# OCR-D/ocrd_keraslm

Hardware: AMD Instinct MI355X
Metric: chars/sec training (stacked-LSTM forward+backward+Adam) (higher is better)
Workload: dtype bf16; 1 GPU; cfg2: depth=2 width=512 length=256 V=256 1 context, stateful training, 3072 streams/GPU, synthetic 10M-char corpus (SURVEY.md 8d); streams_per_gpu=3072, global_batch=3072, seq_len=256, parallelism=dp1

## Files before the change

include/keraslm_hip.h:

```cpp
#ifndef KERASLM_HIP_H
#define KERASLM_HIP_H

#include <stddef.h>
#include <stdint.h>

#ifdef __cplusplus
extern "C" {
#endif

#define KL_ABI_VERSION 1

enum {
  KL_OK = 0,
  KL_ERR_SHAPE = 1,
  KL_ERR_LAUNCH = 2,
  KL_ERR_STATE = 3,
  KL_ERR_WORKSPACE = 4,
  KL_ERR_ARG = 5
};

#define KL_PREC_BF16 1
#define KL_PREC_SPLIT 3

typedef struct kl_config {
// ... 44 lines not shown
int kl_step_batch(kl_handle* h, int n, const int32_t* idx, const int32_t* ctx, float* pool, const int32_t* slot_in,
                  const int32_t* slot_out, float* probs, void* ws, size_t ws_bytes, void* stream);

void* kl_host_alloc(size_t bytes);
void kl_host_free(void* p);
size_t kl_step_host_workspace_bytes(const kl_handle* h, int n);
int kl_step_batch_host(kl_handle* h, int n, const int32_t* idx, const int32_t* ctx, const int32_t* slot_in,
                       const int32_t* slot_out, const int32_t* target, float* pool, int head_k, float* probs_host,
                       float* heads_host, uint32_t* done_host, uint32_t ticket, void* ws, size_t ws_bytes, void* stream);
int kl_step_wait(const uint32_t* done_host, uint32_t ticket, double timeout_s);

int kl_state_dist2(const kl_handle* h, int n, const float* pool, const int32_t* a, const int32_t* b, int k,
                   float* out, void* stream);

int kl_trace_enable(kl_handle* h, int on);
int kl_trace_read(kl_handle* h, int kind, int* n_launches, float* total_ms, int* persistent,
                  double* flops_per_launch);
const char* kl_trace_kernel_name(kl_handle* h, int kind);

int kl_test_gemm_tn(const uint16_t* A, const uint16_t* B, void* C, const float* bias, int M, int N, int K, long lda,
                    long ldb, long ldc, int out_mode, int splits, void* stream);
int kl_test_gemm_an(const uint16_t* A_km, const uint16_t* B, float* C, int M, int N, int K, long lda_km, long ldb,
                    long ldc, int c_transposed, int b_km, void* stream);
int kl_test_thin_gemm(const float* A, long lda, const uint16_t* WT_hi, const uint16_t* WT_lo, long ldw, int M, int N,
                      int K, float* C, long ldc, int split, void* stream);

#ifdef __cplusplus
}
#endif
#endif
```

ocrd_keraslm_amd/csrc/api.hip:

```cpp
#include <hip/hip_runtime.h>
#include <stdio.h>
#include <stdlib.h>
#include <string.h>
#include <time.h>

#include <functional>
#include <utility>

#include <vector>

#include "kl_common.h"
#include "kl_kernels.h"

namespace {

inline size_t align_up(size_t x, size_t a) { return (x + a - 1) / a * a; }
inline int round_up_i(int x, int a) { return (x + a - 1) / a * a; }

struct Carver {
  unsigned char* base;
  size_t off = 0;
  explicit Carver(void* b) : base(reinterpret_cast<unsigned char*>(b)) {}
  template <typename T>
  T* take(size_t count) {
// ... 1205 lines not shown
    } else if (dz_km) {
      KL_TRY(kl_launch_gemm_an(w.dZ[l], (const bf16_t*)w.H[l], grads + h->off_U[l], 4 * W, W, BT, 4 * W, W, 4 * W, 1, s, 1));
    } else if (w.ht_ready) {
      KL_TRY(kl_launch_gemm_tn(w.HTf[l], w.dZT, grads + h->off_U[l], nullptr, W, 4 * W, BT, ldtf, BTp, 4 * W, 2, ksplit, 1.f, s));
    } else {
      KL_TRY(kl_launch_transpose_bf16((const bf16_t*)w.H[l], W, w.HT, BTp, BT, W, s));
      KL_TRY(kl_launch_gemm_tn(w.HT, w.dZT, grads + h->off_U[l], nullptr, W, 4 * W, BTp, BTp, BTp, 4 * W, 2, ksplit, 1.f, s));
    }
    if (!db_done) KL_TRY(kl_launch_colsum_bf16(w.dZ[l], 4 * W, BT, 4 * W, grads + h->off_b[l], s));
    if (l > 0) {
      const bool masked_in = masks != nullptr && (l - 1) > 0;
      const bf16_t* X = masked_in ? w.Hd[l - 1] : (const bf16_t*)w.H[l - 1] + BW;
      if (pair_uk) {
      } else if (dz_km) {
        KL_TRY(kl_launch_gemm_an(w.dZ[l], X, grads + h->off_K[l], 4 * W, W, BT, 4 * W, W, 4 * W, 1, s, 1));
      } else if (w.ht_ready) {
        const bf16_t* XT = masked_in ? w.HdT[l - 1] : w.HTf[l - 1] + B;
        KL_TRY(kl_launch_gemm_tn(XT, w.dZT, grads + h->off_K[l], nullptr, W, 4 * W, BT, masked_in ? (long)BT : ldtf, BTp, 4 * W, 2, ksplit, 1.f, s));
      } else {
        KL_TRY(kl_launch_transpose_bf16(X, W, w.HT, BTp, BT, W, s));
        KL_TRY(kl_launch_gemm_tn(w.HT, w.dZT, grads + h->off_K[l], nullptr, W, 4 * W, BTp, BTp, BTp, 4 * W, 2, ksplit, 1.f, s));
      }
    } else {
      if (kl_launch_onehot_dense(idx, B, T, Vp, 0, 1, w.OHT, BTp, s) == KL_ERR_SHAPE) {
        KL_TRY(kl_zero_async(w.OHT, (size_t)Vp * BTp * sizeof(bf16_t), s));
        KL_TRY(kl_launch_onehot_t(idx, B, T, V, 0, 1, w.OHT, BTp, s));
      }
      KL_TRY(kl_zero_async(w.dEKT, (size_t)4 * W * Vp * sizeof(float), s));
      bool pair_ctx = dz_km && h->fuse_wg && c.n_ctx >= 1 && (Vp % 128) == 0 &&
                      kl_gemm_an_applicable(4 * W, Vp + c.ctx_vocab, BT, 4 * W);
      if (pair_ctx) {
        if (kl_launch_onehot_dense(ctx, B, T, c.ctx_vocab, 0, c.n_ctx, w.OHC[0], BTp, s) == KL_ERR_SHAPE) {
          KL_TRY(kl_zero_async(w.OHC[0], (size_t)c.ctx_vocab * BTp * sizeof(bf16_t), s));
          KL_TRY(kl_launch_onehot_t(ctx, B, T, c.ctx_vocab, 0, c.n_ctx, w.OHC[0], BTp, s));
        }
        KL_TRY(kl_zero_async(w.dCtxKT[0], (size_t)4 * W * c.ctx_vocab * sizeof(float), s));
        const int pe = kl_launch_gemm_an2(w.dZ[l], w.OHT, w.dEKT, 4 * W, Vp, BT, 4 * W, BTp, Vp, 0,
                                          w.OHC[0], w.dCtxKT[0], c.ctx_vocab, BTp, c.ctx_vocab, 0, s, 0);
        if (pe == KL_ERR_SHAPE) pair_ctx = false;
        else KL_TRY(pe);
      }
      if (pair_ctx) {
      } else if (dz_km) KL_TRY(kl_launch_gemm_an(w.dZ[l], w.OHT, w.dEKT, 4 * W, Vp, BT, 4 * W, BTp, Vp, 0, s));
      else KL_TRY(kl_launch_gemm_tn(w.dZT, w.OHT, w.dEKT, nullptr, 4 * W, Vp, BTp, BTp, BTp, Vp, 2, ksplit, 1.f, s));
      KL_TRY(kl_launch_f32_to_bf16_t(w.dEKT, Vp, 4 * W, Vp, w.dEKT_bf, nullptr, Vp, 0, s));
      KL_TRY(kl_launch_f32_to_bf16_t(w.dEKT, Vp, 4 * W, Vp, w.dEK_bf, nullptr, 4 * W, 1, s));
      KL_TRY(kl_launch_gemm_tn(d.ET, w.dEKT_bf, grads + h->off_K[0], nullptr, W, 4 * W, Vp, Vp, Vp, 4 * W, 0, 1, 1.f, s));
      KL_TRY(kl_launch_gemm_tn(w.dEK_bf, d.Kn[0], grads + h->off_E, nullptr, V, W, 4 * W, 4 * W, 4 * W, W, 2, 1, 1.f, s));
      for (int n = 0; n < c.n_ctx; ++n) {
        if (!(pair_ctx && n == 0)) {
          if (kl_launch_onehot_dense(ctx, B, T, c.ctx_vocab, n, c.n_ctx, w.OHC[n], BTp, s) == KL_ERR_SHAPE) {
            KL_TRY(kl_zero_async(w.OHC[n], (size_t)c.ctx_vocab * BTp * sizeof(bf16_t), s));
            KL_TRY(kl_launch_onehot_t(ctx, B, T, c.ctx_vocab, n, c.n_ctx, w.OHC[n], BTp, s));
          }
          KL_TRY(kl_zero_async(w.dCtxKT[n], (size_t)4 * W * c.ctx_vocab * sizeof(float), s));
          if (dz_km) KL_TRY(kl_launch_gemm_an(w.dZ[l], w.OHC[n], w.dCtxKT[n], 4 * W, c.ctx_vocab, BT, 4 * W, BTp, c.ctx_vocab, 0, s));
          else KL_TRY(kl_launch_gemm_tn(w.dZT, w.OHC[n], w.dCtxKT[n], nullptr, 4 * W, c.ctx_vocab, BTp, BTp, BTp,
                                        c.ctx_vocab, 2, ksplit, 1.f, s));
        }
        const size_t krow = (size_t)(W + n * c.ctx_dim) * 4 * W;
        KL_TRY(kl_launch_ctx_grads(P + h->off_Ctx[n], P + h->off_K[0] + krow, 4 * W, c.ctx_vocab, c.ctx_dim,
                                   w.dCtxKT[n], c.ctx_vocab, 4 * W, grads + h->off_K[0] + krow, 4 * W,
                                   grads + h->off_Ctx[n], s));
      }
    }
      return 0;
// ... 538 lines not shown
  }
}

int kl_state_dist2(const kl_handle* h, int n, const float* pool, const int32_t* a, const int32_t* b, int k, float* out,
                   void* stream) {
  if (!h || !pool || !a || !b || !out || n < 1) return KL_ERR_ARG;
  if (k < 0 || k >= 2 * h->cfg.depth) return KL_ERR_ARG;
  const int W = h->cfg.width;
  hipLaunchKernelGGL(state_dist2_kernel, dim3((n + 3) / 4), dim3(256), 0, (hipStream_t)stream, pool,
                     (long)2 * h->cfg.depth * W, W, k, a, b, n, out);
  return hip_ok(hipGetLastError());
}

int kl_test_gemm_tn(const uint16_t* A, const uint16_t* B, void* C, const float* bias, int M, int N, int K, long lda,
                    long ldb, long ldc, int out_mode, int splits, void* stream) {
  return kl_launch_gemm_tn(A, B, C, bias, M, N, K, lda, ldb, ldc, out_mode, splits, 1.f, (hipStream_t)stream);
}

int kl_test_gemm_an(const uint16_t* A_km, const uint16_t* B, float* C, int M, int N, int K, long lda_km, long ldb,
                    long ldc, int c_transposed, int b_km, void* stream) {
  return kl_launch_gemm_an(A_km, B, C, M, N, K, lda_km, ldb, ldc, c_transposed, (hipStream_t)stream, b_km);
}

int kl_test_thin_gemm(const float* A, long lda, const uint16_t* WT_hi, const uint16_t* WT_lo, long ldw, int M, int N,
                      int K, float* C, long ldc, int split, void* stream) {
  KlOperand op;
  memset(&op, 0, sizeof(op));
  op.A = A; op.lda = lda; op.a_is_f32 = 1; op.WT_hi = WT_hi; op.WT_lo = WT_lo; op.ldw = ldw; op.K = K;
  return kl_launch_thin_gemm(&op, M, N, C, ldc, nullptr, split, (hipStream_t)stream);
}

}

extern "C" int kl_test_fwd_step(const uint16_t* A, long lda, const uint16_t* WT, long ldw, int K, int n_ops,
                                int n_rows, int W, int fused, int iters, float* c_out, uint16_t* h_out,
                                void* stream) {
  KlFwdStep st[4];
  if (fused < 1 || fused > 4 || n_ops < 1 || n_ops > 2) return KL_ERR_ARG;
  for (int f = 0; f < fused; ++f) {
    KlFwdStep& S = st[f];
    memset(&S, 0, sizeof(S));
    S.n_rows = n_rows; S.W = W; S.split = 1; S.n_ops = n_ops;
    for (int p = 0; p < n_ops; ++p) {
      KlOperand& o = S.op[p];
      o.A = A; o.lda = lda; o.WT_hi = WT + (size_t)(f * 2 + p) * (size_t)4 * W * ldw; o.ldw = ldw;
      o.K = K; o.a_is_f32 = 0;
// ... 143 lines not shown
```

ocrd_keraslm_amd/csrc/elementwise.hip:

```cpp
#include <string.h>

#include "kl_common.h"
#include "kl_kernels.h"

namespace {

struct CtxTabs { const float* t[8]; };

__global__ void embed_gather_kernel(const float* __restrict__ E, CtxTabs tabs, int n_ctx, int ctx_dim, int W,
                                    const int* __restrict__ idx, const int* __restrict__ ctx, int B, int T,
                                    bf16_t* __restrict__ X, long ldx, int Dp) {
  const int chunks = Dp >> 3;
  const long total = (long)B * T * chunks;
  for (long e = blockIdx.x * (long)blockDim.x + threadIdx.x; e < total; e += (long)gridDim.x * blockDim.x) {
    const int c = (int)(e % chunks);
    const long row = e / chunks;
    const int b = (int)(row % B), t = (int)(row / B);
    const int id = idx[(long)b * T + t];
    frag16 o;
#pragma unroll
    for (int j = 0; j < 8; ++j) {
      const int d = c * 8 + j;
      float v = 0.f;
      if (d < W) {
// ... 272 lines not shown
                                    bf16_t* __restrict__ out, long ld) {
  const long r0 = ((long)blockIdx.x * blockDim.x + threadIdx.x) * 8;
  if (r0 >= ld) return;
  const long total = (long)B * T;
  int id[8];
#pragma unroll
  for (int j = 0; j < 8; ++j) {
    const long r = r0 + j;
    id[j] = -1;
    if (r < total) {
      const int b = (int)(r % B), t = (int)(r / B);
      id[j] = ids[((long)b * T + t) * n_cols + col];
    }
  }
  const int v0 = blockIdx.y * 32;
  for (int v = v0; v < v0 + 32 && v < n_rows; ++v) {
    uint4 w;
    w.x = (id[0] == v ? 0x3F80u : 0u) | (id[1] == v ? 0x3F800000u : 0u);
    w.y = (id[2] == v ? 0x3F80u : 0u) | (id[3] == v ? 0x3F800000u : 0u);
    w.z = (id[4] == v ? 0x3F80u : 0u) | (id[5] == v ? 0x3F800000u : 0u);
    w.w = (id[6] == v ? 0x3F80u : 0u) | (id[7] == v ? 0x3F800000u : 0u);
    *reinterpret_cast<uint4*>(out + (long)v * ld + r0) = w;
  }
}

__global__ void reg_stats_kernel(const float* __restrict__ X, int R, int D, float* __restrict__ scratch) {
  extern __shared__ float sm[];
  float* col = sm;
  float* red = sm + D;
  const int tid = threadIdx.x, nt = blockDim.x;
  float* mean = scratch;
  float* s1 = scratch + D;
  float* s2 = scratch + 2 * D;
  float* nr = scratch + 3 * D;
  for (int d = tid; d < D; d += nt) col[d] = 0.f;
  __syncthreads();
  if (D <= nt) {
    const int ng = nt / D, g = tid / D, d = tid % D;
    if (g < ng) {
      float a = 0.f;
#pragma unroll 8
      for (int r = 1 + g; r < R; r += ng) a += X[(long)r * D + d];
      atomicAdd(&col[d], a);
    }
  } else {
    for (int d = tid; d < D; d += nt) {
// ... 204 lines not shown

int kl_launch_adam(float* p, const float* g, float* m, float* v, size_t n, float lr_t, float b1, float b2,
                   float eps, float clip, float grad_scale, hipStream_t stream) {
  hipLaunchKernelGGL(adam_kernel, dim3(grid_for((long)n, 256)), dim3(256), 0, stream, p, g, m, v, n, lr_t, b1, b2,
                     eps, clip, grad_scale);
  return ok();
}

int kl_launch_onehot_t(const int* ids, int B, int T, int n_classes, int col, int n_cols, bf16_t* out, long ld,
                       hipStream_t stream) {
  hipLaunchKernelGGL(onehot_t_kernel, dim3(grid_for((long)B * T, 256)), dim3(256), 0, stream, ids, B, T, n_classes,
                     col, n_cols, out, ld);
  return ok();
}

int kl_launch_onehot_dense(const int* ids, int B, int T, int n_rows, int col, int n_cols, bf16_t* out, long ld,
                           hipStream_t stream) {
  if ((ld & 7) || ((size_t)out & 15) || ld < (long)B * T) return KL_ERR_SHAPE;
  dim3 grid((unsigned)((ld / 8 + 255) / 256), (unsigned)((n_rows + 31) / 32));
  hipLaunchKernelGGL(onehot_dense_kernel, grid, dim3(256), 0, stream, ids, B, T, n_rows, col, n_cols, out, ld);
  return ok();
}

int kl_launch_regulariser_grads(const float* E, int V, int W, const float* const* ctx_tabs, int n_ctx, int ctx_vocab,
                                int ctx_dim, float* gE, float* const* gCtx, float* loss_acc, float* scratch,
                                hipStream_t stream) {
  const int nt = 1024;
  if (V >= 2) {
    const size_t lds = (size_t)(W + 2 * nt) * sizeof(float);
    if (lds > 64 * 1024) return KL_ERR_SHAPE;
    hipLaunchKernelGGL(reg_stats_kernel, dim3(1), dim3(nt), lds, stream, E, V, W, scratch);
    hipLaunchKernelGGL(reg_apply_kernel, dim3(grid_for((long)V * W, 256)), dim3(256), 0, stream, E, V, W, gE, 0, scratch,
                       loss_acc);
  }
  for (int n = 0; n < n_ctx; ++n) {
    const size_t lds = (size_t)(ctx_dim + 2 * nt) * sizeof(float);
    hipLaunchKernelGGL(reg_stats_kernel, dim3(1), dim3(nt), lds, stream, ctx_tabs[n], ctx_vocab, ctx_dim, scratch);
    hipLaunchKernelGGL(reg_apply_kernel, dim3(grid_for((long)ctx_vocab * ctx_dim, 256)), dim3(256), 0, stream, ctx_tabs[n],
                       ctx_vocab, ctx_dim, gCtx[n], 1, scratch, loss_acc);
  }
  return ok();
}

int kl_launch_state_to_rows(const float* states, int B, int W, int L, int layer, bf16_t* h_bf16, float* h_f32,
                            float* c_f32, hipStream_t stream) {
  hipLaunchKernelGGL(state_to_rows_kernel, dim3(grid_for((long)B * W, 256)), dim3(256), 0, stream, states, B, W, L,
// ... 80 lines not shown
```

ocrd_keraslm_amd/csrc/gemm.hip:

```cpp
#include <stdlib.h>
#include <string.h>

#include "kl_common.h"
#include "kl_kernels.h"

namespace {

constexpr int BN = 128, BK = 64;
constexpr int NTHREADS = 256;

__device__ __forceinline__ int lds_off(int row, int chunk) {
  return row * 128 + ((chunk ^ ((row >> 1) & 7)) << 4);
}

template <int OUT, int BM>
__global__ __launch_bounds__(NTHREADS) void gemm_tn_kernel(
    const bf16_t* __restrict__ A, const bf16_t* __restrict__ B, void* __restrict__ Cv,
    const float* __restrict__ bias, int M, int N, int K, long lda, long ldb, long ldc,
    int k_per_split, float alpha) {
  constexpr int WM = BM / 64;
  constexpr int WN = 4 / WM;
  constexpr int NT = BN / WN / 16;
  constexpr int ALOADS = BM * 8 / NTHREADS;
  extern __shared__ __attribute__((aligned(16))) unsigned char smem[];
// ... 634 lines not shown
#define KL_LONG_CASE(O)                                                                                                  \
  do {                                                                                                                   \
    static KlLdsGrant grant_a, grant_b;                                                  \
    if (kl_grant_lds(grant_a, reinterpret_cast<const void*>(&gemm_tn_long_kernel<O, true, RF, WM, WN>), lds)) return KL_ERR_LAUNCH;  \
    if (kl_grant_lds(grant_b, reinterpret_cast<const void*>(&gemm_tn_long_kernel<O, false, RF, WM, WN>), lds)) return KL_ERR_LAUNCH; \
    if (ilv) hipLaunchKernelGGL((gemm_tn_long_kernel<O, true, RF, WM, WN>), grid, dim3(64 * WM * WN), lds, stream, A, B, C,  \
                                bias, M, N, K, lda, ldb, ldc, k_per_split, alpha, epi, remap, 0, KlGemmSecond{});                        \
    else hipLaunchKernelGGL((gemm_tn_long_kernel<O, false, RF, WM, WN>), grid, dim3(64 * WM * WN), lds, stream, A, B, C,     \
                            bias, M, N, K, lda, ldb, ldc, k_per_split, alpha, epi, remap, 0, KlGemmSecond{});                            \
  } while (0)
  if (out_mode == 0) KL_LONG_CASE(0);
  else if (out_mode == 1) KL_LONG_CASE(1);
  else if (out_mode == 3) KL_LONG_CASE(3);
  else KL_LONG_CASE(2);
#undef KL_LONG_CASE
  return 0;
}

int launch_long(int out_mode, dim3 grid, hipStream_t stream, const bf16_t* A, const bf16_t* B, void* C, const float* bias,
                int M, int N, int K, long lda, long ldb, long ldc, int k_per_split, float alpha) {
  return launch_long_t<4, 4, 2>(out_mode, grid, stream, A, B, C, bias, M, N, K, lda, ldb, ldc, k_per_split, alpha);
}

}

int kl_launch_gemm_tn(const bf16_t* A, const bf16_t* B, void* C, const float* bias, int M, int N, int K,
                      long lda, long ldb, long ldc, int out_mode, int splits, float alpha, hipStream_t stream) {
  if (M <= 0 || N <= 0 || K <= 0) return 0;
  if ((K & 7) || (lda & 7) || (ldb & 7)) return KL_ERR_SHAPE;
  if (splits < 1) splits = 1;
  if (out_mode != 2) splits = 1;
  static const int long_mode = getenv("KL_GEMM_LONG") ? atoi(getenv("KL_GEMM_LONG")) : 2;
  const bool long_ok = (K % BK) == 0 && lda < (1L << 22) && ldb < (1L << 22);
  if (long_mode >= 1 && long_ok && out_mode == 2 && K >= 8192) {
    const int tiles = ((M + LBM - 1) / LBM) * ((N + LBN - 1) / LBN);
    int sp = (256 + tiles - 1) / tiles;
    const int nk = K / BK;
    if (sp > nk / 16) sp = nk / 16;
    if (sp < 1) sp = 1;
    const int kps = ((nk + sp - 1) / sp) * BK;
    sp = (K + kps - 1) / kps;
    dim3 grid((N + LBN - 1) / LBN, (M + LBM - 1) / LBM, sp);
    const int e = launch_long(out_mode, grid, stream, A, B, C, bias, M, N, K, lda, ldb, ldc, kps, alpha);
    if (e != 0) return e;
    return hipGetLastError() == hipSuccess ? 0 : KL_ERR_LAUNCH;
  }
// ... 40 lines not shown
    launch_bm<64>(out_mode, grid, stream, A, B, C, bias, M, N, K, lda, ldb, ldc, k_per_split, alpha);
  } else {
    dim3 grid(nbx, (M + 127) / 128, splits);
    launch_bm<128>(out_mode, grid, stream, A, B, C, bias, M, N, K, lda, ldb, ldc, k_per_split, alpha);
  }
  return hipGetLastError() == hipSuccess ? 0 : KL_ERR_LAUNCH;
}

static int an_rows_per_split(int M, int n_all, int K, long ld_max) {
  if (M <= 0 || n_all <= 0 || K <= 0 || (M % LBM) || (K % BK)) return 0;
  const int tiles = (M / LBM) * ((n_all + LBN - 1) / LBN);
  int sp = (256 + tiles - 1) / tiles;
  const int nk = K / BK;
  if (sp > nk / 16) sp = nk / 16;
  if (sp < 1) sp = 1;
  int kps = ((nk + sp - 1) / sp) * BK;
  while ((long)kps * ld_max * 2 >= 0x7fffffffL && kps > BK) {
    ++sp;
    kps = ((nk + sp - 1) / sp) * BK;
  }
  return (long)kps * ld_max * 2 < 0x7fffffffL ? kps : 0;
}

bool kl_gemm_an_applicable(int M, int N, int K, long lda_km) {
  if (lda_km & 7) return false;
  return an_rows_per_split(M, N, K, lda_km) > 0;
}

int kl_launch_gemm_an2(const bf16_t* A_km, const bf16_t* B, float* C, int M, int N, int K, long lda_km, long ldb, long ldc,
                       int c_transposed, const bf16_t* B2, float* C2, int N2, long ldb2, long ldc2, int c_transposed2,
                       hipStream_t stream, int b_km) {
  if (M <= 0 || N <= 0 || K <= 0) return 0;
  if (B2 != nullptr && ((N % LBN) || N2 <= 0 || (ldb2 & 7) || (!b_km && ldb2 >= (1L << 22)))) return KL_ERR_SHAPE;
  const int n_all = B2 != nullptr ? N + N2 : N;
  if ((lda_km & 7) || (ldb & 7) || (!b_km && ldb >= (1L << 22))) return KL_ERR_SHAPE;
  long ld_max = lda_km;
  if (b_km && ldb > ld_max) ld_max = ldb;
  if (b_km && B2 != nullptr && ldb2 > ld_max) ld_max = ldb2;
  const int kps = an_rows_per_split(M, n_all, K, ld_max);
  if (kps <= 0) return KL_ERR_SHAPE;
  const int sp = (K + kps - 1) / kps;
  dim3 grid((n_all + LBN - 1) / LBN, M / LBM, sp);
  KlGateEpi epi;
  memset(&epi, 0, sizeof(epi));
  KlGemmSecond second;
  memset(&second, 0, sizeof(second));
  if (B2 != nullptr) {
    second.B = B2;
    second.C = C2;
    second.n_first = N;
    second.N = N2;
    second.ldb = ldb2;
    second.ldc = ldc2;
    second.c_transposed = c_transposed2;
  }
  const size_t lds = (size_t)LSTAGES * (LBM + LBN) * 128;
  static const int remap = !(getenv("KL_GEMM_XCD") && getenv("KL_GEMM_XCD")[0] == '0');
  static KlLdsGrant grant_a, grant_b;
  if (kl_grant_lds(grant_a, reinterpret_cast<const void*>(&gemm_tn_long_kernel<2, true, 4, 4, 2, true, false>), lds)) return KL_ERR_LAUNCH;
  if (kl_grant_lds(grant_b, reinterpret_cast<const void*>(&gemm_tn_long_kernel<2, true, 4, 4, 2, true, true>), lds)) return KL_ERR_LAUNCH;
  if (b_km)
    hipLaunchKernelGGL((gemm_tn_long_kernel<2, true, 4, 4, 2, true, true>), grid, dim3(512), lds, stream, A_km, B, (void*)C,
                       (const float*)nullptr, M, N, K, lda_km, ldb, ldc, kps, 1.f, epi, remap, c_transposed, second);
  else
    hipLaunchKernelGGL((gemm_tn_long_kernel<2, true, 4, 4, 2, true, false>), grid, dim3(512), lds, stream, A_km, B, (void*)C,
                       (const float*)nullptr, M, N, K, lda_km, ldb, ldc, kps, 1.f, epi, remap, c_transposed, second);
  return hipGetLastError() == hipSuccess ? 0 : KL_ERR_LAUNCH;
}

int kl_launch_gemm_an(const bf16_t* A_km, const bf16_t* B, float* C, int M, int N, int K, long lda_km, long ldb, long ldc,
                      int c_transposed, hipStream_t stream, int b_km) {
  return kl_launch_gemm_an2(A_km, B, C, M, N, K, lda_km, ldb, ldc, c_transposed, nullptr, nullptr, 0, 0, 0, 0, stream, b_km);
}

int kl_launch_gemm_gates(const bf16_t* A3, const bf16_t* WTperm, int n, int W, int Kc, long lda, const KlGateEpi* epi,
                         hipStream_t stream) {
  if (n < 1 || (W & 31) || (Kc % BK) != 0 || (lda & 7) || lda >= (1L << 22) || !epi) return KL_ERR_SHAPE;
  dim3 grid(4 * W / LBN, (n + 63) / 64, 1);
  const int e = launch_long_t<2, 2, 4>(3, grid, stream, A3, WTperm, nullptr, nullptr, n, 4 * W, Kc, lda, lda, 0, Kc, 1.f, epi);
  if (e != 0) return e;
// ... 3 lines not shown
```

ocrd_keraslm_amd/csrc/kl_kernels.h:

```cpp
#pragma once
#include <hip/hip_runtime.h>
#include <stdint.h>

#include "keraslm_hip.h"

typedef unsigned short bf16_t;

#include <atomic>
#include <mutex>
#define KL_MAX_DEVICES 64
struct KlLdsGrant {
  std::atomic<size_t> granted[KL_MAX_DEVICES];
  std::mutex slow;
};
static inline int kl_grant_lds(KlLdsGrant& g, const void* fn, size_t lds) {
  int dev = 0;
  if (hipGetDevice(&dev) != hipSuccess) return KL_ERR_LAUNCH;
  if (dev < 0 || dev >= KL_MAX_DEVICES)
    return hipFuncSetAttribute(fn, hipFuncAttributeMaxDynamicSharedMemorySize, (int)lds) == hipSuccess ? 0 : KL_ERR_LAUNCH;
  if (lds <= g.granted[dev].load(std::memory_order_acquire)) return 0;
  std::lock_guard<std::mutex> lock(g.slow);
  if (lds <= g.granted[dev].load(std::memory_order_relaxed)) return 0;
  if (hipFuncSetAttribute(fn, hipFuncAttributeMaxDynamicSharedMemorySize, (int)lds) != hipSuccess) return KL_ERR_LAUNCH;
  g.granted[dev].store(lds, std::memory_order_release);
// ... 3 lines not shown
struct KlGatherRec {
  const float* pool; long slot_ld; const int* slot_in;
  int n, W, nb;
  bf16_t* out[4];
};
int kl_launch_gather_recurrent(const KlGatherRec& a, int L, hipStream_t stream);
int kl_launch_permute_gate_rows(const bf16_t* src, bf16_t* dst, int W, long cols, hipStream_t stream);

struct KlGateEpi {
  const float* T1; const int* i1;
  const float* T2; const int* i2;
  const float* bias;
  const float* c_prev; long c_ld; const int* slot_in;
  float* c_out; float* h_out; long out_ld; const int* slot_out;
  bf16_t* xn; long ldn; int kn; int nbn;
  int W;
};
int kl_launch_gemm_gates(const bf16_t* A3, const bf16_t* WTperm, int n, int W, int Kc, long lda, const KlGateEpi* epi,
                         hipStream_t stream);

int kl_launch_gemm_tn(const bf16_t* A, const bf16_t* B, void* C, const float* bias, int M, int N, int K,
                      long lda, long ldb, long ldc, int out_mode, int splits, float alpha, hipStream_t stream);
bool kl_gemm_an_applicable(int M, int N, int K, long lda_km);
int kl_launch_gemm_an(const bf16_t* A_km, const bf16_t* B, float* C, int M, int N, int K, long lda_km, long ldb, long ldc,
                      int c_transposed, hipStream_t stream, int b_km = 0);
int kl_launch_gemm_an2(const bf16_t* A_km, const bf16_t* B, float* C, int M, int N, int K, long lda_km, long ldb, long ldc,
                       int c_transposed, const bf16_t* B2, float* C2, int N2, long ldb2, long ldc2, int c_transposed2,
                       hipStream_t stream, int b_km);

struct KlOperand {
  const void* A;
  long lda;
  const int* row_index;
  const bf16_t* WT_hi;
  const bf16_t* WT_lo;
  long ldw;
  int K;
  int a_is_f32;
};

struct KlFwdStep {
  KlOperand op[2];
  int n_ops;
  int n_rows, W;
  int split;
  const float* T1; const int* i1; long t1_ld;
// ... 156 lines not shown
                           hipStream_t stream);
int kl_launch_transpose_bf16(const bf16_t* in, long ld_in, bf16_t* out, long ld_out, int rows, int cols,
                             hipStream_t stream);
#define KL_CONV_MAX_JOBS 24
struct KlConvJob {
  const float* in; long ld_in; int rows, cols, rows_pad, transpose;
  bf16_t* out_hi; bf16_t* out_lo; long ld_out;
};
struct KlConvJobs { KlConvJob job[KL_CONV_MAX_JOBS]; };
int kl_launch_f32_to_bf16_jobs(const KlConvJob* jobs, int n, hipStream_t stream);
int kl_launch_comb_table(const float* A, const float* B, int R1, int R2, int N, bf16_t* out, hipStream_t stream);
int kl_launch_rows_tm(const int* idx, const int* ctx, int n_ctx, int Bn, int T, int R2, int* out, hipStream_t stream);
int kl_launch_f32_to_bf16_t(const float* in, long ld_in, int rows, int cols, bf16_t* out_hi, bf16_t* out_lo,
                            long ld_out, int transpose, hipStream_t stream);
int kl_launch_softmax_ce(float* logits, long ld, int rows, int V, const int* tgt, int B, int T, float inv_count,
                         bf16_t* dlogits, long ld_dl, float* loss_acc, float* rowstat, int time_major,
                         hipStream_t stream, int last_only = 0);
int kl_launch_adam(float* p, const float* g, float* m, float* v, size_t n, float lr_t, float b1, float b2,
                   float eps, float clip, float grad_scale, hipStream_t stream);
int kl_launch_onehot_t(const int* ids, int B, int T, int n_classes, int col, int n_cols, bf16_t* out, long ld,
                       hipStream_t stream);
int kl_launch_onehot_dense(const int* ids, int B, int T, int n_rows, int col, int n_cols, bf16_t* out, long ld,
                           hipStream_t stream);
int kl_launch_regulariser_grads(const float* E, int V, int W, const float* const* ctx_tabs, int n_ctx, int ctx_vocab,
                                int ctx_dim, float* gE, float* const* gCtx, float* loss_acc, float* scratch,
                                hipStream_t stream);
int kl_launch_state_to_rows(const float* states, int B, int W, int L, int layer, bf16_t* h_bf16, float* h_f32,
                            float* c_f32, hipStream_t stream);
int kl_launch_fill_f32(float* p, size_t n, float v, hipStream_t stream);
int kl_launch_fill_bf16(bf16_t* p, size_t n, unsigned short bits, hipStream_t stream);
int kl_zero_async(void* p, size_t bytes, hipStream_t stream);
int kl_fill_u32_async(void* p, size_t bytes, unsigned value, hipStream_t stream);
int kl_zero_coherent_async(unsigned* p, size_t n_words, hipStream_t stream);

int kl_launch_small_table(const float* A, int R, int D, const float* Kmat, long ldk, int N, float* C, long ldc,
                          hipStream_t stream);
int kl_launch_p1_gather(const float* EK, const float* const* ctxk, int n_ctx, const float* bias, const int* idx,
                        const int* ctx, int B, int T, int N, float* P, hipStream_t stream);
int kl_launch_colsum_bf16(const bf16_t* in, long ld, int rows, int cols, float* out, hipStream_t stream);
int kl_launch_rows_to_state(const void* h_rows, int h_is_f32, const float* c_rows, int B, int W, int L, int layer,
                            float* states, hipStream_t stream);
int kl_launch_ctx_grads(const float* Ctx, const float* K0rows, long ldk, int R, int D, const float* dT, long ldt, int N,
                        float* gK, long ldg, float* gCtx, hipStream_t stream);
int kl_launch_rows_tm_to_bm(const float* in, long ld_in, float* out, int B, int T, int V, hipStream_t stream);

#define KL_SMALL_STEP_N 16
// ... 40 lines not shown
```

ocrd_keraslm_amd/lib/hipabi.py:

```python
from __future__ import annotations

import ctypes as C
import os

_HERE = os.path.dirname(os.path.abspath(__file__))
LIB_PATH = os.environ.get("KL_LIB") or os.path.join(os.path.dirname(_HERE), "libkeraslm_hip.so")

KL_PREC_BF16 = 1
KL_PREC_SPLIT = 3


class KlConfig(C.Structure):
    _fields_ = [("depth", C.c_int32), ("width", C.c_int32), ("voc_size", C.c_int32),
                ("n_ctx", C.c_int32), ("ctx_vocab", C.c_int32), ("ctx_dim", C.c_int32)]


class KlError(RuntimeError):
    pass


SIGNATURES = {
    "kl_abi_version": (C.c_int, []),
    "kl_error_string": (C.c_char_p, [C.c_int]),
    "kl_param_count": (C.c_size_t, [C.POINTER(KlConfig)]),
# ... 15 lines not shown
                                     C.c_float, C.c_float, C.c_float, C.c_void_p]),
    "kl_step_workspace_bytes": (C.c_size_t, [C.c_void_p, C.c_int]),
    "kl_step_batch": (C.c_int, [C.c_void_p, C.c_int, C.c_void_p, C.c_void_p, C.c_void_p, C.c_void_p, C.c_void_p,
                                C.c_void_p, C.c_void_p, C.c_size_t, C.c_void_p]),
    "kl_host_alloc": (C.c_void_p, [C.c_size_t]),
    "kl_host_free": (None, [C.c_void_p]),
    "kl_step_host_workspace_bytes": (C.c_size_t, [C.c_void_p, C.c_int]),
    "kl_step_batch_host": (C.c_int, [C.c_void_p, C.c_int, C.c_void_p, C.c_void_p, C.c_void_p, C.c_void_p, C.c_void_p,
                                     C.c_void_p, C.c_int, C.c_void_p, C.c_void_p, C.c_void_p, C.c_uint32, C.c_void_p,
                                     C.c_size_t, C.c_void_p]),
    "kl_step_wait": (C.c_int, [C.c_void_p, C.c_uint32, C.c_double]),
    "kl_state_dist2": (C.c_int, [C.c_void_p, C.c_int, C.c_void_p, C.c_void_p, C.c_void_p, C.c_int, C.c_void_p,
                                 C.c_void_p]),
    "kl_trace_enable": (C.c_int, [C.c_void_p, C.c_int]),
    "kl_set_window_mode": (C.c_int, [C.c_void_p, C.c_int]),
    "kl_set_loss_rows": (C.c_int, [C.c_void_p, C.c_int]),
    "kl_trace_kernel_name": (C.c_char_p, [C.c_void_p, C.c_int]),
    "kl_trace_read": (C.c_int, [C.c_void_p, C.c_int, C.POINTER(C.c_int), C.POINTER(C.c_float), C.POINTER(C.c_int),
                                C.POINTER(C.c_double)]),
    "kl_test_gemm_tn": (C.c_int, [C.c_void_p, C.c_void_p, C.c_void_p, C.c_void_p, C.c_int, C.c_int, C.c_int,
                                  C.c_long, C.c_long, C.c_long, C.c_int, C.c_int, C.c_void_p]),
    "kl_test_gemm_an": (C.c_int, [C.c_void_p, C.c_void_p, C.c_void_p, C.c_int, C.c_int, C.c_int, C.c_long, C.c_long,
                                  C.c_long, C.c_int, C.c_int, C.c_void_p]),
    "kl_test_thin_gemm": (C.c_int, [C.c_void_p, C.c_long, C.c_void_p, C.c_void_p, C.c_long, C.c_int, C.c_int,
                                    C.c_int, C.c_void_p, C.c_long, C.c_int, C.c_void_p]),
}

_lib = None


def load():
    global _lib
    if _lib is not None:
        return _lib
    if not os.path.exists(LIB_PATH):
        raise KlError("HIP extension %s not built: run `make -C ocrd_keraslm_amd/csrc` "
                      "(the Rater has no CPU fallback)" % LIB_PATH)
    lib = C.CDLL(LIB_PATH)
    for name, (res, args) in SIGNATURES.items():
        fn = getattr(lib, name)
        fn.restype = res
        fn.argtypes = args
    _lib = lib
    return lib


# ... 5 lines not shown
```

Before: 34.17 million chars/s.

## Add 256x256 k-major AN GEMM and k-major one-hot for embedding gradient

Adds a new 256x256-tile, 5-stage LDS-ring bf16 MFMA kernel for the A-k-major times B-k-major GEMM, with split-K atomics and XCD remapping, and routes the layer-0 embedding/context weight-gradient GEMM to it. To feed it, the one-hot input is now built directly in k-major (row per timestep) layout by a new vectorised kernel, which avoids the transposed one-hot layout and its zero-fill. The aim is to make the embedding-gradient GEMM more efficient. In exchange there is a large amount of new hand-scheduled kernel code, higher LDS use per block, and atomic output contention when splitting over K.

Result: no change. 34.41 million chars/s, median of 6 (+0.7%).

```diff
diff --git a/include/keraslm_hip.h b/include/keraslm_hip.h
--- a/include/keraslm_hip.h
+++ b/include/keraslm_hip.h
@@ -90,6 +90,11 @@
                     long ldb, long ldc, int out_mode, int splits, void* stream);
 int kl_test_gemm_an(const uint16_t* A_km, const uint16_t* B, float* C, int M, int N, int K, long lda_km, long ldb,
                     long ldc, int c_transposed, int b_km, void* stream);
+int kl_test_gemm_an2(const uint16_t* A_km, const uint16_t* B, float* C, int M, int N, int K, long lda_km, long ldb,
+                     long ldc, int c_transposed, const uint16_t* B2, float* C2, int N2, long ldb2, long ldc2,
+                     int c_transposed2, int b_km, void* stream);
+int kl_test_onehot(const int* ids, int B, int T, int n_rows, int col, int n_cols, uint16_t* out, long ld, int k_major,
+                   void* stream);
 int kl_test_thin_gemm(const float* A, long lda, const uint16_t* WT_hi, const uint16_t* WT_lo, long ldw, int M, int N,
                       int K, float* C, long ldc, int split, void* stream);
 
diff --git a/ocrd_keraslm_amd/csrc/api.hip b/ocrd_keraslm_amd/csrc/api.hip
--- a/ocrd_keraslm_amd/csrc/api.hip
+++ b/ocrd_keraslm_amd/csrc/api.hip
@@ -1251,14 +1251,22 @@
         KL_TRY(kl_launch_gemm_tn(w.HT, w.dZT, grads + h->off_K[l], nullptr, W, 4 * W, BTp, BTp, BTp, 4 * W, 2, ksplit, 1.f, s));
       }
     } else {
-      if (kl_launch_onehot_dense(idx, B, T, Vp, 0, 1, w.OHT, BTp, s) == KL_ERR_SHAPE) {
+      bool pair_ctx = dz_km && h->fuse_wg && c.n_ctx >= 1 && (Vp % 128) == 0 &&
+                      kl_gemm_an_applicable(4 * W, Vp + c.ctx_vocab, BT, 4 * W);
+      const bool oh_km = dz_km && kl_gemm_an256_takes(4 * W, Vp, BT, 4 * W, Vp, pair_ctx ? c.ctx_vocab : 0, c.ctx_vocab);
+      if (oh_km) {
+        KL_TRY(kl_launch_onehot_km(idx, B, T, Vp, 0, 1, w.OHT, Vp, s));
+      } else if (kl_launch_onehot_dense(idx, B, T, Vp, 0, 1, w.OHT, BTp, s) == KL_ERR_SHAPE) {
         KL_TRY(kl_zero_async(w.OHT, (size_t)Vp * BTp * sizeof(bf16_t), s));
         KL_TRY(kl_launch_onehot_t(idx, B, T, V, 0, 1, w.OHT, BTp, s));
       }
       KL_TRY(kl_zero_async(w.dEKT, (size_t)4 * W * Vp * sizeof(float), s));
-      bool pair_ctx = dz_km && h->fuse_wg && c.n_ctx >= 1 && (Vp % 128) == 0 &&
-                      kl_gemm_an_applicable(4 * W, Vp + c.ctx_vocab, BT, 4 * W);
-      if (pair_ctx) {
+      if (pair_ctx && oh_km) {
+        KL_TRY(kl_launch_onehot_km(ctx, B, T, c.ctx_vocab, 0, c.n_ctx, w.OHC[0], c.ctx_vocab, s));
+        KL_TRY(kl_zero_async(w.dCtxKT[0], (size_t)4 * W * c.ctx_vocab * sizeof(float), s));
+        KL_TRY(kl_launch_gemm_an2(w.dZ[l], w.OHT, w.dEKT, 4 * W, Vp, BT, 4 * W, Vp, Vp, 0,
+                                  w.OHC[0], w.dCtxKT[0], c.ctx_vocab, c.ctx_vocab, c.ctx_vocab, 0, s, 1));
+      } else if (pair_ctx) {
         if (kl_launch_onehot_dense(ctx, B, T, c.ctx_vocab, 0, c.n_ctx, w.OHC[0], BTp, s) == KL_ERR_SHAPE) {
           KL_TRY(kl_zero_async(w.OHC[0], (size_t)c.ctx_vocab * BTp * sizeof(bf16_t), s));
           KL_TRY(kl_launch_onehot_t(ctx, B, T, c.ctx_vocab, 0, c.n_ctx, w.OHC[0], BTp, s));
@@ -1270,7 +1278,8 @@
         else KL_TRY(pe);
       }
       if (pair_ctx) {
-      } else if (dz_km) KL_TRY(kl_launch_gemm_an(w.dZ[l], w.OHT, w.dEKT, 4 * W, Vp, BT, 4 * W, BTp, Vp, 0, s));
+      } else if (oh_km) KL_TRY(kl_launch_gemm_an(w.dZ[l], w.OHT, w.dEKT, 4 * W, Vp, BT, 4 * W, Vp, Vp, 0, s, 1));
+      else if (dz_km) KL_TRY(kl_launch_gemm_an(w.dZ[l], w.OHT, w.dEKT, 4 * W, Vp, BT, 4 * W, BTp, Vp, 0, s));
       else KL_TRY(kl_launch_gemm_tn(w.dZT, w.OHT, w.dEKT, nullptr, 4 * W, Vp, BTp, BTp, BTp, Vp, 2, ksplit, 1.f, s));
       KL_TRY(kl_launch_f32_to_bf16_t(w.dEKT, Vp, 4 * W, Vp, w.dEKT_bf, nullptr, Vp, 0, s));
       KL_TRY(kl_launch_f32_to_bf16_t(w.dEKT, Vp, 4 * W, Vp, w.dEK_bf, nullptr, 4 * W, 1, s));
@@ -1855,6 +1864,19 @@
   return kl_launch_gemm_an(A_km, B, C, M, N, K, lda_km, ldb, ldc, c_transposed, (hipStream_t)stream, b_km);
 }
 
+int kl_test_gemm_an2(const uint16_t* A_km, const uint16_t* B, float* C, int M, int N, int K, long lda_km, long ldb,
+                     long ldc, int c_transposed, const uint16_t* B2, float* C2, int N2, long ldb2, long ldc2,
+                     int c_transposed2, int b_km, void* stream) {
+  return kl_launch_gemm_an2(A_km, B, C, M, N, K, lda_km, ldb, ldc, c_transposed, B2, C2, N2, ldb2, ldc2, c_transposed2,
+                            (hipStream_t)stream, b_km);
+}
+
+int kl_test_onehot(const int* ids, int B, int T, int n_rows, int col, int n_cols, uint16_t* out, long ld, int k_major,
+                   void* stream) {
+  return k_major ? kl_launch_onehot_km(ids, B, T, n_rows, col, n_cols, out, ld, (hipStream_t)stream)
+                 : kl_launch_onehot_dense(ids, B, T, n_rows, col, n_cols, out, ld, (hipStream_t)stream);
+}
+
 int kl_test_thin_gemm(const float* A, long lda, const uint16_t* WT_hi, const uint16_t* WT_lo, long ldw, int M, int N,
                       int K, float* C, long ldc, int split, void* stream) {
   KlOperand op;
diff --git a/ocrd_keraslm_amd/csrc/elementwise.hip b/ocrd_keraslm_amd/csrc/elementwise.hip
--- a/ocrd_keraslm_amd/csrc/elementwise.hip
+++ b/ocrd_keraslm_amd/csrc/elementwise.hip
@@ -318,6 +318,24 @@
     w.w = (id[6] == v ? 0x3F80u : 0u) | (id[7] == v ? 0x3F800000u : 0u);
     *reinterpret_cast<uint4*>(out + (long)v * ld + r0) = w;
   }
+}
+
+__global__ void onehot_km_kernel(const int* __restrict__ ids, int B, int T, int n_rows, int col, int n_cols,
+                                 bf16_t* __restrict__ out, long ld) {
+  const long q = (long)blockIdx.x * blockDim.x + threadIdx.x;
+  const long per_row = ld / 8;
+  const long r = q / per_row;
+  if (r >= (long)B * T) return;
+  const int v0 = (int)(q - r * per_row) * 8;
+  const int b = (int)(r % B), t = (int)(r / B);
+  const int id = ids[((long)b * T + t) * n_cols + col];
+  const int d = id < n_rows ? id - v0 : -1;
+  uint4 w;
+  w.x = (d == 0 ? 0x3F80u : 0u) | (d == 1 ? 0x3F800000u : 0u);
+  w.y = (d == 2 ? 0x3F80u : 0u) | (d == 3 ? 0x3F800000u : 0u);
+  w.z = (d == 4 ? 0x3F80u : 0u) | (d == 5 ? 0x3F800000u : 0u);
+  w.w = (d == 6 ? 0x3F80u : 0u) | (d == 7 ? 0x3F800000u : 0u);
+  *reinterpret_cast<uint4*>(out + r * ld + v0) = w;
 }
 
 __global__ void reg_stats_kernel(const float* __restrict__ X, int R, int D, float* __restrict__ scratch) {
@@ -568,6 +586,15 @@
   return ok();
 }
 
+int kl_launch_onehot_km(const int* ids, int B, int T, int n_rows, int col, int n_cols, bf16_t* out, long ld,
+                        hipStream_t stream) {
+  if ((ld & 7) || ((size_t)out & 15) || ld < n_rows) return KL_ERR_SHAPE;
+  const long threads = (long)B * T * (ld / 8);
+  hipLaunchKernelGGL(onehot_km_kernel, dim3((unsigned)((threads + 255) / 256)), dim3(256), 0, stream, ids, B, T, n_rows,
+                     col, n_cols, out, ld);
+  return ok();
+}
+
 int kl_launch_regulariser_grads(const float* E, int V, int W, const float* const* ctx_tabs, int n_ctx, int ctx_vocab,
                                 int ctx_dim, float* gE, float* const* gCtx, float* loss_acc, float* scratch,
                                 hipStream_t stream) {
diff --git a/ocrd_keraslm_amd/csrc/gemm.hip b/ocrd_keraslm_amd/csrc/gemm.hip
--- a/ocrd_keraslm_amd/csrc/gemm.hip
+++ b/ocrd_keraslm_amd/csrc/gemm.hip
@@ -680,6 +680,177 @@
   return launch_long_t<4, 4, 2>(out_mode, grid, stream, A, B, C, bias, M, N, K, lda, ldb, ldc, k_per_split, alpha);
 }
 
+constexpr int AN_BM = 256, AN_BN = 256, AN_BK = 32, AN_STAGES = 5;
+constexpr int AN_STAGE_BYTES = (AN_BM + AN_BN) * AN_BK * 2;
+
+template <int NS>
+__global__ __launch_bounds__(512, 1) void gemm_an256_kernel(
+    const bf16_t* __restrict__ A, const bf16_t* __restrict__ B_, float* __restrict__ C_, int M, int N_, int K, long lda,
+    long ldb_, long ldc_, int k_per_split, int xcd_remap, int c_t_, const KlGemmSecond second) {
+  constexpr int WN = 2, RF = 4, NT = 8;
+  constexpr int PA = 2, PB = 2, NP = PA + PB;
+  constexpr int A_BYTES = AN_BM * AN_BK * 2;
+  const bf16_t* __restrict__ B = B_;
+  float* __restrict__ Cv = C_;
+  int N = N_, c_t = c_t_;
+  long ldb = ldb_, ldc = ldc_;
+  extern __shared__ __attribute__((aligned(16))) unsigned char smem[];
+  const int tid = threadIdx.x;
+  const int lane = tid & 63;
+  const int wave = __builtin_amdgcn_readfirstlane(tid >> 6);
+  const int wm = wave / WN, wn = wave % WN;
+  int bx = blockIdx.x, by = blockIdx.y, bz = blockIdx.z;
+  {
+    const unsigned nx = gridDim.x, ny = gridDim.y, total = nx * ny * gridDim.z;
+    if (xcd_remap && (total & 7) == 0) {
+      const unsigned lin = bx + nx * (by + ny * bz);
+      const unsigned re = (lin & 7) * (total >> 3) + (lin >> 3);
+      bx = re % nx;
+      by = (re / nx) % ny;
+      bz = re / (nx * ny);
+    }
+  }
+  const int m0 = by * AN_BM;
+  int n0 = bx * AN_BN;
+  if (second.B != nullptr) {
+    if (n0 >= second.n_first) {
+      n0 -= second.n_first;
+      B = second.B;
+      Cv = reinterpret_cast<float*>(second.C);
+      N = second.N;
+      ldb = second.ldb;
+      ldc = second.ldc;
+      c_t = second.c_transposed;
+    } else {
+      N = second.n_first;
+    }
+  }
+  const int kbeg = bz * k_per_split;
+  const int kend = min(K, kbeg + k_per_split);
+  const int nkt = (kend - kbeg) / AN_BK;
+
+  auto clamp31 = [](long v) { return (int)(v > 0x7fffffffL ? 0x7fffffffL : (v < 0 ? 0 : v)); };
+  const __amdgpu_buffer_rsrc_t rsA = __builtin_amdgcn_make_buffer_rsrc(
+      const_cast<bf16_t*>(A + (long)kbeg * lda + m0), 0, clamp31(((long)(kend - kbeg - 1) * lda + (M - m0)) * 2), 0x00020000);
+  const __amdgpu_buffer_rsrc_t rsB = __builtin_amdgcn_make_buffer_rsrc(
+      const_cast<bf16_t*>(B + (long)kbeg * ldb + n0), 0, clamp31(((long)(kend - kbeg - 1) * ldb + (N - n0)) * 2), 0x00020000);
+  unsigned vo[NP];
+#pragma unroll
+  for (int j = 0; j < NP; ++j) {
+    const int krow = 2 * (wave * 2 + (j & 1)) + (lane >> 5);
+    const int c = (lane & 31) ^ (2 * ((krow & 3) | (((krow >> 3) & 1) << 2)));
+    vo[j] = (unsigned)((long)krow * (j < PA ? lda : ldb) * 2 + c * 16);
+  }
+  const unsigned lds0 = (unsigned)(size_t)(lds_void_t*)smem;
+  auto issue = [&](int kt, int stage) {
+    const int soff_a = (int)((long)kt * AN_BK * lda * 2);
+    const int soff_b = (int)((long)kt * AN_BK * ldb * 2);
+    const unsigned sa = lds0 + stage * AN_STAGE_BYTES + wave * PA * 1024;
+    const unsigned sb = lds0 + stage * AN_STAGE_BYTES + A_BYTES + wave * PB * 1024;
+#pragma unroll
+    for (int j = 0; j < PA; ++j) glds16(rsA, vo[j], soff_a, sa + j * 1024);
+#pragma unroll
+    for (int j = 0; j < PB; ++j) glds16(rsB, vo[PA + j], soff_b, sb + j * 1024);
+  };
+
+  f32x4 acc[RF][NT];
+#pragma unroll
+  for (int i = 0; i < RF; ++i)
+#pragma unroll
+    for (int j = 0; j < NT; ++j) acc[i][j] = f32x4{0.f, 0.f, 0.f, 0.f};
+
+  const int fr = lane & 15, fq = lane >> 4;
+  unsigned a_off[RF], b_off[NT];
+  {
+    const int q = fr >> 2, pp = fr & 3;
+    const int fl = 2 * (q | ((fq & 1) << 2));
+    const int rb = (fq * 8 + q) * 512 + (pp >> 1) * 16 + 8 * (pp & 1);
+#pragma unroll
+    for (int i = 0; i < RF; ++i) a_off[i] = (unsigned)(rb + (((wm * 64 + i * 16) >> 3) ^ fl) * 16);
+#pragma unroll
+    for (int j = 0; j < NT; ++j) b_off[j] = (unsigned)(A_BYTES + rb + (((wn * 128 + j * 16) >> 3) ^ fl) * 16);
+  }
+  auto read_frags = [&](int stage, frag16 (&fa)[RF], frag16 (&fb)[NT]) {
+    const unsigned char* base = smem + stage * AN_STAGE_BYTES;
+#pragma unroll
+    for (int i = 0; i < RF; ++i) {
+      const unsigned char* ap = base + a_off[i];
+      const s16x4 lo = __builtin_amdgcn_ds_read_tr16_b64_v4i16((lds_s16x4*)(ap));
+      const s16x4 hi = __builtin_amdgcn_ds_read_tr16_b64_v4i16((lds_s16x4*)(ap + 4 * 512));
+      fa[i].v = __builtin_bit_cast(bf16x8, __builtin_shufflevector(lo, hi, 0, 1, 2, 3, 4, 5, 6, 7));
+    }
+#pragma unroll
+    for (int j = 0; j < NT; ++j) {
+      const unsigned char* bp = base + b_off[j];
+      const s16x4 lo = __builtin_amdgcn_ds_read_tr16_b64_v4i16((lds_s16x4*)(bp));
+      const s16x4 hi = __builtin_amdgcn_ds_read_tr16_b64_v4i16((lds_s16x4*)(bp + 4 * 512));
+      fb[j].v = __builtin_bit_cast(bf16x8, __builtin_shufflevector(lo, hi, 0, 1, 2, 3, 4, 5, 6, 7));
+    }
+  };
+  auto wait_landed = [](int ahead) {
+    if (ahead >= 3) asm volatile("s_waitcnt vmcnt(%0)" ::"n"(3 * NP) : "memory");
+    else if (ahead == 2) asm volatile("s_waitcnt vmcnt(%0)" ::"n"(2 * NP) : "memory");
+    else if (ahead == 1) asm volatile("s_waitcnt vmcnt(%0)" ::"n"(NP) : "memory");
+    else asm volatile("s_waitcnt vmcnt(0)" ::: "memory");
+  };
+  static_assert(NS >= 3 && NS <= 5, "ring depth");
+
+  frag16 fa0[RF], fb0[NT], fa1[RF], fb1[NT];
+#pragma unroll
+  for (int p = 0; p < NS - 1; ++p)
+    if (p < nkt) issue(p, p);
+  if (nkt > 0) {
+    wait_landed(min(nkt - 1, NS - 2));
+    __builtin_amdgcn_s_barrier();
+    read_frags(0, fa0, fb0);
+  }
+  auto step = [&](int kt, int stage, frag16 (&fa)[RF], frag16 (&fb)[NT], frag16 (&ga)[RF], frag16 (&gb)[NT]) {
+    __builtin_amdgcn_s_waitcnt(0xC07F);
+    __builtin_amdgcn_sched_barrier(0);
+    __builtin_amdgcn_s_setprio(1);
+#pragma unroll
+    for (int i = 0; i < RF; ++i)
+#pragma unroll
+      for (int j = 0; j < NT / 2; ++j) acc[i][j] = mfma16(fa[i].v, fb[j].v, acc[i][j]);
+    __builtin_amdgcn_s_setprio(0);
+    __builtin_amdgcn_sched_barrier(0);
+    if (kt + 1 < nkt) {
+      wait_landed(min(nkt - 2 - kt, NS - 3));
+      __builtin_amdgcn_s_barrier();
+      if (kt + NS - 1 < nkt) issue(kt + NS - 1, stage >= 1 ? stage - 1 : NS - 1);
+      read_frags(stage + 1 < NS ? stage + 1 : 0, ga, gb);
+    }
+    __builtin_amdgcn_sched_barrier(0);
+    __builtin_amdgcn_s_setprio(1);
+#pragma unroll
+    for (int i = 0; i < RF; ++i)
+#pragma unroll
+      for (int j = NT / 2; j < NT; ++j) acc[i][j] = mfma16(fa[i].v, fb[j].v, acc[i][j]);
+    __builtin_amdgcn_s_setprio(0);
+  };
+  int stage = 0;
+  for (int kt = 0; kt < nkt; kt += 2) {
+    step(kt, stage, fa0, fb0, fa1, fb1);
+    stage = stage + 1 < NS ? stage + 1 : 0;
+    if (kt + 1 < nkt) step(kt + 1, stage, fa1, fb1, fa0, fb0);
+    stage = stage + 1 < NS ? stage + 1 : 0;
+  }
+#pragma unroll
+  for (int i = 0; i < RF; ++i) {
+#pragma unroll
+    for (int j = 0; j < NT; ++j) {
+      const int col = n0 + wn * 128 + j * 16 + fr;
+      if (col >= N) continue;
+#pragma unroll
+      for (int r = 0; r < 4; ++r) {
+        const int row = m0 + wm * 64 + i * 16 + fq * 4 + r;
+        if (c_t) atomicAdd(Cv + (long)col * ldc + row, acc[i][j][r]);
+        else atomicAdd(Cv + (long)row * ldc + col, acc[i][j][r]);
+      }
+    }
+  }
+}
+
 }
 
 int kl_launch_gemm_tn(const bf16_t* A, const bf16_t* B, void* C, const float* bias, int M, int N, int K,
@@ -766,15 +937,70 @@
   return (long)kps * ld_max * 2 < 0x7fffffffL ? kps : 0;
 }
 
+static int an256_rows_per_split(int M, int n_all, int K, long ld_max) {
+  if (M <= 0 || n_all <= 0 || K <= 0 || (M % AN_BM) || (K % AN_BK)) return 0;
+  const int tiles = (M / AN_BM) * ((n_all + AN_BN - 1) / AN_BN);
+  int sp = (256 + tiles - 1) / tiles;
+  const int nk = K / AN_BK;
+  if (sp > nk / 16) sp = nk / 16;
+  if (sp < 1) return 0;
+  int kps = ((nk + sp - 1) / sp) * AN_BK;
+  while ((long)kps * ld_max * 2 >= 0x7fffffffL && kps > AN_BK) {
+    ++sp;
+    kps = ((nk + sp - 1) / sp) * AN_BK;
+  }
+  return (long)kps * ld_max * 2 < 0x7fffffffL ? kps : 0;
+}
+
+static bool an256_enabled() {
+  static const bool on = !(getenv("KL_GEMM_AN256") && getenv("KL_GEMM_AN256")[0] == '0');
+  return on;
+}
+
+static int an256_plan(int M, int N, int K, long lda_km, long ldb, int N2, long ldb2, int b_km) {
+  if (!an256_enabled() || !b_km || (lda_km & 7) || (ldb & 7)) return 0;
+  if (N2 > 0 && ((N % AN_BN) || (ldb2 & 7))) return 0;
+  long ld_max = lda_km > ldb ? lda_km : ldb;
+  if (N2 > 0 && ldb2 > ld_max) ld_max = ldb2;
+  return an256_rows_per_split(M, N2 > 0 ? N + N2 : N, K, ld_max);
+}
+
 bool kl_gemm_an_applicable(int M, int N, int K, long lda_km) {
   if (lda_km & 7) return false;
   return an_rows_per_split(M, N, K, lda_km) > 0;
+}
+
+bool kl_gemm_an256_takes(int M, int N, int K, long lda_km, long ldb, int N2, long ldb2) {
+  return an256_plan(M, N, K, lda_km, ldb, N2, ldb2, 1) > 0;
 }
 
 int kl_launch_gemm_an2(const bf16_t* A_km, const bf16_t* B, float* C, int M, int N, int K, long lda_km, long ldb, long ldc,
                        int c_transposed, const bf16_t* B2, float* C2, int N2, long ldb2, long ldc2, int c_transposed2,
                        hipStream_t stream, int b_km) {
   if (M <= 0 || N <= 0 || K <= 0) return 0;
+  KlGemmSecond second;
+  memset(&second, 0, sizeof(second));
+  if (B2 != nullptr) {
+    second.B = B2;
+    second.C = C2;
+    second.n_first = N;
+    second.N = N2;
+    second.ldb = ldb2;
+    second.ldc = ldc2;
+    second.c_transposed = c_transposed2;
+  }
+  static const int remap = !(getenv("KL_GEMM_XCD") && getenv("KL_GEMM_XCD")[0] == '0');
+  const int kps256 = an256_plan(M, N, K, lda_km, ldb, B2 != nullptr ? N2 : 0, ldb2, b_km);
+  if (kps256 > 0) {
+    const int n_all = B2 != nullptr ? N + N2 : N;
+    dim3 grid((n_all + AN_BN - 1) / AN_BN, M / AN_BM, (K + kps256 - 1) / kps256);
+    const size_t lds = (size_t)AN_STAGES * AN_STAGE_BYTES;
+    static KlLdsGrant grant;
+    if (kl_grant_lds(grant, reinterpret_cast<const void*>(&gemm_an256_kernel<AN_STAGES>), lds)) return KL_ERR_LAUNCH;
+    hipLaunchKernelGGL((gemm_an256_kernel<AN_STAGES>), grid, dim3(512), lds, stream, A_km, B, C, M, N, K, lda_km, ldb, ldc,
+                       kps256, remap, c_transposed, second);
+    return hipGetLastError() == hipSuccess ? 0 : KL_ERR_LAUNCH;
+  }
   if (B2 != nullptr && ((N % LBN) || N2 <= 0 || (ldb2 & 7) || (!b_km && ldb2 >= (1L << 22)))) return KL_ERR_SHAPE;
   const int n_all = B2 != nullptr ? N + N2 : N;
   if ((lda_km & 7) || (ldb & 7) || (!b_km && ldb >= (1L << 22))) return KL_ERR_SHAPE;
@@ -787,19 +1013,7 @@
   dim3 grid((n_all + LBN - 1) / LBN, M / LBM, sp);
   KlGateEpi epi;
   memset(&epi, 0, sizeof(epi));
-  KlGemmSecond second;
-  memset(&second, 0, sizeof(second));
-  if (B2 != nullptr) {
-    second.B = B2;
-    second.C = C2;
-    second.n_first = N;
-    second.N = N2;
-    second.ldb = ldb2;
-    second.ldc = ldc2;
-    second.c_transposed = c_transposed2;
-  }
   const size_t lds = (size_t)LSTAGES * (LBM + LBN) * 128;
-  static const int remap = !(getenv("KL_GEMM_XCD") && getenv("KL_GEMM_XCD")[0] == '0');
   static KlLdsGrant grant_a, grant_b;
   if (kl_grant_lds(grant_a, reinterpret_cast<const void*>(&gemm_tn_long_kernel<2, true, 4, 4, 2, true, false>), lds)) return KL_ERR_LAUNCH;
   if (kl_grant_lds(grant_b, reinterpret_cast<const void*>(&gemm_tn_long_kernel<2, true, 4, 4, 2, true, true>), lds)) return KL_ERR_LAUNCH;
diff --git a/ocrd_keraslm_amd/csrc/kl_kernels.h b/ocrd_keraslm_amd/csrc/kl_kernels.h
--- a/ocrd_keraslm_amd/csrc/kl_kernels.h
+++ b/ocrd_keraslm_amd/csrc/kl_kernels.h
@@ -49,6 +49,7 @@
 int kl_launch_gemm_tn(const bf16_t* A, const bf16_t* B, void* C, const float* bias, int M, int N, int K,
                       long lda, long ldb, long ldc, int out_mode, int splits, float alpha, hipStream_t stream);
 bool kl_gemm_an_applicable(int M, int N, int K, long lda_km);
+bool kl_gemm_an256_takes(int M, int N, int K, long lda_km, long ldb, int N2, long ldb2);
 int kl_launch_gemm_an(const bf16_t* A_km, const bf16_t* B, float* C, int M, int N, int K, long lda_km, long ldb, long ldc,
                       int c_transposed, hipStream_t stream, int b_km = 0);
 int kl_launch_gemm_an2(const bf16_t* A_km, const bf16_t* B, float* C, int M, int N, int K, long lda_km, long ldb, long ldc,
@@ -251,6 +252,8 @@
                        hipStream_t stream);
 int kl_launch_onehot_dense(const int* ids, int B, int T, int n_rows, int col, int n_cols, bf16_t* out, long ld,
                            hipStream_t stream);
+int kl_launch_onehot_km(const int* ids, int B, int T, int n_rows, int col, int n_cols, bf16_t* out, long ld,
+                        hipStream_t stream);
 int kl_launch_regulariser_grads(const float* E, int V, int W, const float* const* ctx_tabs, int n_ctx, int ctx_vocab,
                                 int ctx_dim, float* gE, float* const* gCtx, float* loss_acc, float* scratch,
                                 hipStream_t stream);
diff --git a/ocrd_keraslm_amd/lib/hipabi.py b/ocrd_keraslm_amd/lib/hipabi.py
--- a/ocrd_keraslm_amd/lib/hipabi.py
+++ b/ocrd_keraslm_amd/lib/hipabi.py
@@ -61,6 +61,11 @@
                                   C.c_long, C.c_long, C.c_long, C.c_int, C.c_int, C.c_void_p]),
     "kl_test_gemm_an": (C.c_int, [C.c_void_p, C.c_void_p, C.c_void_p, C.c_int, C.c_int, C.c_int, C.c_long, C.c_long,
                                   C.c_long, C.c_int, C.c_int, C.c_void_p]),
+    "kl_test_gemm_an2": (C.c_int, [C.c_void_p, C.c_void_p, C.c_void_p, C.c_int, C.c_int, C.c_int, C.c_long, C.c_long,
+                                   C.c_long, C.c_int, C.c_void_p, C.c_void_p, C.c_int, C.c_long, C.c_long, C.c_int,
+                                   C.c_int, C.c_void_p]),
+    "kl_test_onehot": (C.c_int, [C.c_void_p, C.c_int, C.c_int, C.c_int, C.c_int, C.c_int, C.c_void_p, C.c_long, C.c_int,
+                                 C.c_void_p]),
     "kl_test_thin_gemm": (C.c_int, [C.c_void_p, C.c_long, C.c_void_p, C.c_void_p, C.c_long, C.c_int, C.c_int,
                                     C.c_int, C.c_void_p, C.c_long, C.c_int, C.c_void_p]),
 }
```
